# Lemok00/IDEAS

Measured on AMD Instinct MI355X. Metric: train images/sec at 256x256 (G+D+Ex step), higher is better.
Workload: dtype f32; 1 GPU; IDEAS N=1 sigma=1 256x256 batch=32/GPU full G+D+Ex iteration (lazy R1 every 16, EMA), full-width nets, HIP kernels (BASELINE.json configs[2]); global_batch=32, parallelism=dp1, r1_steps_in_window=0, ranks=1

## Files before the change

### ideas_amd/csrc/conv_b3_wgrad3.hip

```cpp
#include "b3.hpp"
#include "conv_launch.hpp"

ideas_plan ideas_b3_wgrad3_plan(const ideas_conv_params* p, int, int64_t slots) {
    if (slots <= 0) slots = 512;
    const int64_t tiles = (int64_t)(p->Cout / 64) * (p->Cin / 64), strips = p->OW / 16, rows_total = (int64_t)p->B * p->OH;
    const int64_t spl = std::min(splitk_target(slots, tiles * strips, rows_total, 128), std::max<int64_t>(rows_total / 16, 1));
    const SplitK k = splitk_round(rows_total, spl, 1);
    return {{k.splits * strips, k.per}, slots};
}

namespace {

typedef short s16x4 __attribute__((ext_vector_type(4)));
typedef short s16x8 __attribute__((ext_vector_type(8)));

template <int S> struct W3 {
    static constexpr int XW = 15 * S + 3;
    static constexpr int NR = 4;
    static constexpr int XROWS = NR * XW;
    static constexpr int GROWS = 2 * 16;
    static constexpr int XPLANE = XROWS * 128, GPLANE = GROWS * 128;
    static constexpr int LDS = 3 * (XPLANE + GPLANE);
    static constexpr int XLOADS = (XW * 16 + 255) / 256;
};


template <int S, bool SCALE, bool REFLECT>
__global__ __launch_bounds__(256, 2) void conv_b3_wgrad3_kernel(float* __restrict__ gw, const float* __restrict__ gy,
                                                                const float* __restrict__ x, const float* __restrict__ in_scale,
                                                                const float* __restrict__ out_scale, ideas_conv_params p,
                                                                int tiles_ci, int tiles, int splits, int strips, int rows_per_split,
                                                                unsigned gy_bytes, unsigned x_bytes) {
    using L = W3<S>;
    constexpr int XW = L::XW, NR = L::NR;
    __shared__ __attribute__((aligned(16))) unsigned char smem[L::LDS];
    unsigned char* const sG = smem;
    unsigned char* const sX = smem + 3 * L::GPLANE;

    const int t = threadIdx.x, lane = t & 63, wave = t >> 6;
    int tile, split;
    splitk_xcd_map(blockIdx.x, tiles, splits, tile, split);
    const int o0 = (tile / tiles_ci) * 64, c0 = (tile % tiles_ci) * 64;
    const int strip = split % strips, range = split / strips;
    const int ox0 = strip * 16;
    const int rows_total = p.B * p.OH;
    const int R0 = range * rows_per_split;
    const int R1 = R0 + rows_per_split < rows_total ? R0 + rows_per_split : rows_total;
    if (R0 >= R1) return;

    const __amdgpu_buffer_rsrc_t rg = __builtin_amdgcn_make_buffer_rsrc((void*)gy, 0, (int)gy_bytes, (int)RSRC_FLAGS);
    const __amdgpu_buffer_rsrc_t rx = __builtin_amdgcn_make_buffer_rsrc((void*)x, 0, (int)x_bytes, (int)RSRC_FLAGS);
    const __amdgpu_buffer_rsrc_t rso = __builtin_amdgcn_make_buffer_rsrc((void*)out_scale, 0, SCALE ? p.B * p.Cout * 4 : 0, (int)RSRC_FLAGS);
    const __amdgpu_buffer_rsrc_t rsi = __builtin_amdgcn_make_buffer_rsrc((void*)in_scale, 0, SCALE ? p.B * p.Cin * 4 : 0, (int)RSRC_FLAGS);

    const int quad = t & 15, px = t >> 4;
    const unsigned g_cb = (unsigned)(o0 + quad * 4) * 4u, x_cb = (unsigned)(c0 + quad * 4) * 4u;
    auto xrow_of = [](int j) { return S == 1 ? j : (j & 1) * 17 + (j >> 1); };
    int x_lrow[L::XLOADS];
    bool x_on[L::XLOADS];
#pragma unroll
    for (int k = 0; k < L::XLOADS; ++k) {
        const int j = px + 16 * k;
        x_on[k] = j < XW;
        x_lrow[k] = xrow_of(j < XW ? j : 0);
    }

    struct Task { int b, wy, oy; bool mma, live; };
    int tk_b, tk_oa, tk_ob, tk_wy, tk_g;
    bool tk_done = false;
    {
        tk_g = R0;
        tk_b = R0 / p.OH;
        tk_oa = R0 - tk_b * p.OH;
        const int left = R1 - R0;
        tk_ob = tk_oa + left < p.OH ? tk_oa + left : p.OH;
        tk_wy = tk_oa * S;
    }
    auto next_task = [&]() -> Task {
        Task k;
        k.live = !tk_done;
        k.b = tk_b;
        k.wy = tk_wy;
        const int rel = tk_wy - tk_oa * S;
        k.mma = k.live && rel >= 2 && ((rel - 2) % S == 0);
        k.oy = tk_oa + (rel - 2) / S;
        if (!tk_done) {
            ++tk_wy;
            if (tk_wy > (tk_ob - 1) * S + 2) {
                tk_g += tk_ob - tk_oa;
                if (tk_g >= R1) tk_done = true;
                else {
                    ++tk_b;
                    tk_oa = 0;
                    tk_ob = R1 - tk_g < p.OH ? R1 - tk_g : p.OH;
                    tk_wy = 0;
                }
            }
        }
        return k;
    };

    struct Stage { float4 g, xv[L::XLOADS], sg, sx; };
    auto gload = [&](Stage& st, const Task& k) {
        int iy = k.wy + p.offy;
        bool yok = k.live;
        if (REFLECT) iy = reflect_coord(iy, p.IH);
        else yok = yok && (unsigned)iy < (unsigned)p.IH;
        const unsigned rowb = (unsigned)((k.b * p.IH + iy) * p.IW) * (unsigned)p.Cin * 4u + x_cb;
#pragma unroll
        for (int q = 0; q < L::XLOADS; ++q) {
            int ix = ox0 * S + p.offx + px + 16 * q;
            bool ok = yok && x_on[q];
            if (REFLECT) ix = reflect_coord(ix, p.IW);
            else ok = ok && (unsigned)ix < (unsigned)p.IW;
            st.xv[q] = buffer_load4(rx, ok ? rowb + (unsigned)ix * (unsigned)p.Cin * 4u : 0xffffffffu, 0);
        }
        const unsigned goff = (unsigned)(((k.b * p.OH + k.oy) * p.OW + ox0 + px) * p.Cout) * 4u + g_cb;
        st.g = buffer_load4(rg, k.mma ? goff : 0xffffffffu, 0);
        if (SCALE) {
            st.sg = buffer_load4(rso, (unsigned)(k.b * p.Cout) * 4u + g_cb, 0);
            st.sx = buffer_load4(rsi, (unsigned)(k.b * p.Cin) * 4u + x_cb, 0);
        }
    };
    auto put = [&](unsigned char* plane0, int plane_bytes, int row, float4 v, float4 sc) {
        if (SCALE) v = b3_scale4(v, sc);
        const Split4 s = split4(v);
        unsigned char* a = plane0 + chunk_off(row, quad >> 1) + (quad & 1) * 8;
#pragma unroll
        for (int pl = 0; pl < 3; ++pl) *reinterpret_cast<uint2*>(a + pl * plane_bytes) = s.p[pl];
    };
    auto lstore = [&](const Stage& st, int n) {
        const int slot = n % NR;
#pragma unroll
        for (int q = 0; q < L::XLOADS; ++q)
            if (x_on[q]) put(sX, L::XPLANE, slot * XW + x_lrow[q], st.xv[q], st.sx);
        put(sG, L::GPLANE, (n & 1) * 16 + px, st.g, st.sg);
    };

    const int wo = wave >> 1, wc = wave & 1;
    const int li = lane & 31, lh = lane >> 5;
    const int g_q = lane & 15, g_row = g_q >> 2, g_piece = g_q & 3, g_cblk = (lane >> 4) & 1;
    auto lane_base = [&](unsigned region, int b, int cb) {
        const int r = b + 8 * lh + g_row;
        return region + (unsigned)(r * 128 + (((cb * 2 + (g_piece >> 1)) ^ ((((b + g_row) >> 1) & 1) << 2)) << 4) + (g_piece & 1) * 8);
    };
    const unsigned ldsG = (unsigned)(uintptr_t)(__attribute__((address_space(3))) unsigned char*)sG;
    const unsigned ldsX = (unsigned)(uintptr_t)(__attribute__((address_space(3))) unsigned char*)sX;
    unsigned baseG[4], baseX[4];
#pragma unroll
    for (int b = 0; b < 4; ++b) { baseG[b] = lane_base(ldsG, b, wo * 2 + g_cblk); baseX[b] = lane_base(ldsX, b, wc * 2 + g_cblk); }
    auto tr_ld = [&](unsigned addr) -> s16x4 {
        return __builtin_amdgcn_ds_read_tr16_b64_v4i16((__attribute__((address_space(3))) s16x4*)(uintptr_t)addr);
    };
    auto frag = [&](const unsigned (&base)[4], int plane_off, int r0) -> bf16x8 {
        const unsigned a0 = base[r0 & 3] + (unsigned)(plane_off + (r0 & ~3) * 128);
        const s16x4 a = tr_ld(a0);
        const s16x4 b = tr_ld(a0 + 512u);
        const s16x8 v = {a[0], a[1], a[2], a[3], b[0], b[1], b[2], b[3]};
        return __builtin_bit_cast(bf16x8, v);
    };

    f32x16 acc[9];
#pragma unroll
    for (int a = 0; a < 9; ++a)
#pragma unroll
        for (int r = 0; r < 16; ++r) acc[a][r] = 0.f;

    auto compute = [&](auto ph_) {
        constexpr int PH = decltype(ph_)::value;
        bf16x8 fa[3];
#pragma unroll
        for (int pl = 0; pl < 3; ++pl) fa[pl] = frag(baseG, pl * L::GPLANE, (PH & 1) * 16);
        auto loadB = [&](int tap, bf16x8 (&fb)[3]) {
            const int ty = tap / 3, tx = tap - 3 * ty;
            const int r0 = ((PH + 2 + ty) % NR) * XW + (S == 1 ? tx : (tx & 1) * 17 + (tx >> 1));
#pragma unroll
            for (int pl = 0; pl < 3; ++pl) fb[pl] = frag(baseX, pl * L::XPLANE, r0);
        };
        bf16x8 fb[5][2][3];
        loadB(0, fb[0][0]);
        loadB(1, fb[0][1]);
#pragma unroll
        for (int pr = 0; pr < 5; ++pr) {
            if (pr < 4) {
                loadB(2 * pr + 2, fb[pr + 1][0]);
                if (2 * pr + 3 < 9) loadB(2 * pr + 3, fb[pr + 1][1]);
            }
            __builtin_amdgcn_sched_barrier(0);
#pragma unroll
            for (int q = 0; q < 6; ++q) {
                acc[2 * pr] = __builtin_amdgcn_mfma_f32_32x32x16_bf16(fa[PA[q]], fb[pr][0][PB[q]], acc[2 * pr], 0, 0, 0);
                if (2 * pr + 1 < 9)
                    acc[2 * pr + 1] = __builtin_amdgcn_mfma_f32_32x32x16_bf16(fa[PA[q]], fb[pr][1][PB[q]], acc[2 * pr + 1], 0, 0, 0);
            }
            __builtin_amdgcn_sched_barrier(0);
        }
    };

    Stage st0, st1;
    Task k0 = next_task();
    gload(st0, k0);
    Task k1 = next_task();
    gload(st1, k1);
    lstore(st0, 0);
    __syncthreads();
    bool mma0 = k0.mma, mma1 = k1.mma, live0 = k0.live, live1 = k1.live;
    static_assert(NR == 4, "the step loop is unrolled over the ring positions");
    auto step = [&](auto ph_, Stage& ld, const Stage& stg) {
        constexpr int PH = decltype(ph_)::value;
        const Task k2 = next_task();
        gload(ld, k2);
        if (live1) lstore(stg, PH + 1);
        if (mma0) compute(ph_);
        __syncthreads();
        mma0 = mma1; live0 = live1; mma1 = k2.mma; live1 = k2.live;
    };
    while (live0) {
        step(std::integral_constant<int, 0>{}, st0, st1);
        if (!live0) break;
        step(std::integral_constant<int, 1>{}, st1, st0);
        if (!live0) break;
        step(std::integral_constant<int, 2>{}, st0, st1);
        if (!live0) break;
        step(std::integral_constant<int, 3>{}, st1, st0);
    }

    const int ci = c0 + wc * 32 + li;
#pragma unroll
    for (int tap = 0; tap < 9; ++tap)
#pragma unroll
        for (int r = 0; r < 16; ++r) {
            const int o = o0 + wo * 32 + (r & 3) + 8 * (r >> 2) + 4 * lh;
            atomicAdd(&gw[((int64_t)o * 9 + tap) * p.Cin + ci], acc[tap][r] * p.gain);
        }
}



template <int S>
int launch_wgrad3(float* gw, const void* gy, const void* x, const float* in_scale, const float* out_scale, const ideas_conv_params* p,
                  hipStream_t stream) {
    const int tiles_ci = p->Cin / 64, tiles = (p->Cout / 64) * tiles_ci;
    const int strips = p->OW / 16;
    const SplitK k = ideas_b3_wgrad3_plan(p, 0, 0).k;
    if (!ideas_grid_fits(tiles * k.splits)) return IDEAS_E_SHAPE;
    with_flags(in_scale && out_scale, p->reflect, [&](auto sc, auto rf) {
        hipLaunchKernelGGL((conv_b3_wgrad3_kernel<S, decltype(sc)::value, decltype(rf)::value>), dim3(splitk_grid(tiles, k.splits)),
                           dim3(256), 0, stream, gw, (const float*)gy, (const float*)x, in_scale, out_scale, *p, tiles_ci, tiles,
                           (int)k.splits, strips, (int)k.per, ideas_gy_bytes(p, 4), ideas_x_bytes(p, 4));
    });
    return ideas_launch_status();
}

}

bool ideas_b3_wgrad3_enabled() { return !ideas_env_off("IDEAS_B3_WGRAD3"); }

extern "C" int ideas_b3_wgrad3_supported(const ideas_conv_params* p) {
    if (!p) return 0;
    if (p->TY != 3 || p->TX != 3 || p->dy != 1 || p->dx != 1 || p->sy != p->sx || (p->sy != 1 && p->sy != 2)) return 0;
    if (p->osy != 1 || p->osx != 1 || p->ooy != 0 || p->oox != 0 || p->YH != p->OH || p->YW != p->OW) return 0;
    if (p->OW % 16 || p->Cin % 64 || p->Cout % 64) return 0;
    if (p->sy == 2 && ideas_env_off("IDEAS_B3_WGRAD3_S2")) return 0;
    if (p->reflect && (p->IH < 2 || p->IW < 2)) return 0;
    if (p->offx > 0 || p->offx < -2 || p->offy > 0 || p->offy < -2) return 0;
    return (int64_t)p->B * p->IH * p->IW * p->Cin * 4 < 0xffffffffLL && (int64_t)p->B * p->YH * p->YW * p->Cout * 4 < 0xffffffffLL &&
           (int64_t)p->B * p->OH < 0x7fffffffLL;
}

int ideas_b3_wgrad3(float* gw, const void* gy, const void* x, const float* in_scale, const float* out_scale, const ideas_conv_params* p,
                    hipStream_t stream) {
    if (p->sy == 1) return launch_wgrad3<1>(gw, gy, x, in_scale, out_scale, p, stream);
    return launch_wgrad3<2>(gw, gy, x, in_scale, out_scale, p, stream);
}
```

Before: 85.74 images/sec.

## Extend 3x3 weight-grad MFMA kernel to narrow widths and 32-channel inputs

Adds new tilings to the 3x3 weight-gradient kernel. Small spatial widths (8 or 4 pixels) pack several images into one 16-pixel strip. Layers with Cin=32 use a pair of 16-pixel strips so the 64-wide tile stays full. Before this, these shapes fell back to a generic weight-grad path. The change adds several template instantiations and layout complexity, and the narrow-width case with scaling still routes to the old kernel.

```diff
diff --git a/ideas_amd/csrc/conv_b3_wgrad3.hip b/ideas_amd/csrc/conv_b3_wgrad3.hip
--- a/ideas_amd/csrc/conv_b3_wgrad3.hip
+++ b/ideas_amd/csrc/conv_b3_wgrad3.hip
@@ -1,9 +1,18 @@
 #include "b3.hpp"
 #include "conv_launch.hpp"
 
+enum { W3_WIDE = 16, W3_PAIR = 32, W3_SEG8 = 8, W3_SEG4 = 4 };
+static int w3_form(const ideas_conv_params* p) {
+    if (p->Cin == 32) return W3_PAIR;
+    return p->OW == 8 ? W3_SEG8 : p->OW == 4 ? W3_SEG4 : W3_WIDE;
+}
+
 ideas_plan ideas_b3_wgrad3_plan(const ideas_conv_params* p, int, int64_t slots) {
     if (slots <= 0) slots = 512;
-    const int64_t tiles = (int64_t)(p->Cout / 64) * (p->Cin / 64), strips = p->OW / 16, rows_total = (int64_t)p->B * p->OH;
+    const int form = w3_form(p);
+    const int64_t tiles = (int64_t)(p->Cout / 64) * (form == W3_PAIR ? 1 : p->Cin / 64);
+    const int64_t strips = form == W3_PAIR ? std::max(p->OW / 32, 1) : form == W3_WIDE ? p->OW / 16 : 1;
+    const int64_t rows_total = (form == W3_SEG8 || form == W3_SEG4 ? (int64_t)p->B / (16 / form) : (int64_t)p->B) * p->OH;
     const int64_t spl = std::min(splitk_target(slots, tiles * strips, rows_total, 128), std::max<int64_t>(rows_total / 16, 1));
     const SplitK k = splitk_round(rows_total, spl, 1);
     return {{k.splits * strips, k.per}, slots};
@@ -14,25 +23,37 @@
 typedef short s16x4 __attribute__((ext_vector_type(4)));
 typedef short s16x8 __attribute__((ext_vector_type(8)));
 
-template <int S> struct W3 {
-    static constexpr int XW = 15 * S + 3;
+template <int S, int SEG = 16, bool PAIR = false> struct W3 {
+    static constexpr int NIMG = 16 / SEG;
+    static constexpr int SW = (SEG - 1) * S + 3;
+    static constexpr int EVEN = SEG + 1;
+    static constexpr int PITCH = (SEG == 4 && S == 1) ? 8 : SW;
+    static constexpr bool BASE2 = SEG == 4 && PITCH % 4 != 0;
+    static constexpr int XW = NIMG * PITCH;
+    static constexpr int XSTAGED = NIMG * SW;
     static constexpr int NR = 4;
     static constexpr int XROWS = NR * XW;
-    static constexpr int GROWS = 2 * 16;
+    static constexpr int GPIX = PAIR ? 32 : 16;
+    static constexpr int GROWS = 2 * GPIX;
     static constexpr int XPLANE = XROWS * 128, GPLANE = GROWS * 128;
     static constexpr int LDS = 3 * (XPLANE + GPLANE);
-    static constexpr int XLOADS = (XW * 16 + 255) / 256;
+    static constexpr int XLOADS = (XSTAGED * 16 + 255) / 256;
+    static_assert(LDS <= 80 * 1024, "two blocks per CU");
 };
 
 
-template <int S, bool SCALE, bool REFLECT>
+template <int S, bool SCALE, bool REFLECT, int SEG = 16, bool PAIR = false>
 __global__ __launch_bounds__(256, 2) void conv_b3_wgrad3_kernel(float* __restrict__ gw, const float* __restrict__ gy,
                                                                 const float* __restrict__ x, const float* __restrict__ in_scale,
                                                                 const float* __restrict__ out_scale, ideas_conv_params p,
                                                                 int tiles_ci, int tiles, int splits, int strips, int rows_per_split,
                                                                 unsigned gy_bytes, unsigned x_bytes) {
-    using L = W3<S>;
+    using L = W3<S, SEG, PAIR>;
     constexpr int XW = L::XW, NR = L::NR;
+    constexpr bool WIDE = SEG == 16 && !PAIR;
+    static_assert(SEG == 16 || SEG == 8 || SEG == 4, "a strip is 16 pixels");
+    static_assert(!PAIR || (SEG == 16 && S == 1), "strip pairs: stride 1");
+    static_assert(SEG == 16 || !SCALE, "image groups: unscaled");
     __shared__ __attribute__((aligned(16))) unsigned char smem[L::LDS];
     unsigned char* const sG = smem;
     unsigned char* const sX = smem + 3 * L::GPLANE;
@@ -42,8 +63,8 @@
     splitk_xcd_map(blockIdx.x, tiles, splits, tile, split);
     const int o0 = (tile / tiles_ci) * 64, c0 = (tile % tiles_ci) * 64;
     const int strip = split % strips, range = split / strips;
-    const int ox0 = strip * 16;
-    const int rows_total = p.B * p.OH;
+    const int ox0 = strip * (PAIR ? 32 : 16);
+    const int rows_total = (SEG < 16 ? p.B / L::NIMG : p.B) * p.OH;
     const int R0 = range * rows_per_split;
     const int R1 = R0 + rows_per_split < rows_total ? R0 + rows_per_split : rows_total;
     if (R0 >= R1) return;
@@ -54,15 +75,34 @@
     const __amdgpu_buffer_rsrc_t rsi = __builtin_amdgcn_make_buffer_rsrc((void*)in_scale, 0, SCALE ? p.B * p.Cin * 4 : 0, (int)RSRC_FLAGS);
 
     const int quad = t & 15, px = t >> 4;
-    const unsigned g_cb = (unsigned)(o0 + quad * 4) * 4u, x_cb = (unsigned)(c0 + quad * 4) * 4u;
-    auto xrow_of = [](int j) { return S == 1 ? j : (j & 1) * 17 + (j >> 1); };
+    const unsigned g_cb = (unsigned)(o0 + quad * 4) * 4u, x_cb = (unsigned)(c0 + (PAIR ? quad & 7 : quad) * 4) * 4u;
+    auto xrow_of = [](int j) { return S == 1 ? j : (j & 1) * L::EVEN + (j >> 1); };
     int x_lrow[L::XLOADS];
     bool x_on[L::XLOADS];
-#pragma unroll
-    for (int k = 0; k < L::XLOADS; ++k) {
-        const int j = px + 16 * k;
-        x_on[k] = j < XW;
-        x_lrow[k] = xrow_of(j < XW ? j : 0);
+    bool x_ok[L::XLOADS];
+    unsigned x_voff[L::XLOADS], g_voff = 0;
+    if constexpr (WIDE) {
+#pragma unroll
+        for (int k = 0; k < L::XLOADS; ++k) {
+            const int j = px + 16 * k;
+            x_on[k] = j < XW;
+            x_lrow[k] = xrow_of(j < XW ? j : 0);
+        }
+    } else {
+#pragma unroll
+        for (int k = 0; k < L::XLOADS; ++k) {
+            const int j = px + 16 * k;
+            x_on[k] = j < L::XSTAGED;
+            const int jj = x_on[k] ? j : 0, img = jj / L::SW, col = jj - img * L::SW;
+            x_lrow[k] = img * L::PITCH + xrow_of(col);
+            int ix = (PAIR ? ox0 + 16 * (quad >> 3) : 0) + p.offx + col;
+            x_ok[k] = x_on[k];
+            if (REFLECT) ix = reflect_coord(ix, p.IW);
+            else x_ok[k] = x_ok[k] && (unsigned)ix < (unsigned)p.IW;
+            x_voff[k] = (unsigned)(img * p.IH * p.IW + ix) * (unsigned)p.Cin * 4u + x_cb;
+        }
+        const int g_pix = PAIR ? ox0 + px : (px / SEG) * p.OH * p.OW + px % SEG;
+        g_voff = (unsigned)(g_pix * p.Cout) * 4u + g_cb;
     }
 
     struct Task { int b, wy, oy; bool mma, live; };
@@ -100,23 +140,33 @@
         return k;
     };
 
-    struct Stage { float4 g, xv[L::XLOADS], sg, sx; };
+    struct Stage { float4 g[PAIR ? 2 : 1], xv[L::XLOADS], sg, sx; };
     auto gload = [&](Stage& st, const Task& k) {
         int iy = k.wy + p.offy;
         bool yok = k.live;
         if (REFLECT) iy = reflect_coord(iy, p.IH);
         else yok = yok && (unsigned)iy < (unsigned)p.IH;
-        const unsigned rowb = (unsigned)((k.b * p.IH + iy) * p.IW) * (unsigned)p.Cin * 4u + x_cb;
-#pragma unroll
-        for (int q = 0; q < L::XLOADS; ++q) {
-            int ix = ox0 * S + p.offx + px + 16 * q;
-            bool ok = yok && x_on[q];
-            if (REFLECT) ix = reflect_coord(ix, p.IW);
-            else ok = ok && (unsigned)ix < (unsigned)p.IW;
-            st.xv[q] = buffer_load4(rx, ok ? rowb + (unsigned)ix * (unsigned)p.Cin * 4u : 0xffffffffu, 0);
-        }
-        const unsigned goff = (unsigned)(((k.b * p.OH + k.oy) * p.OW + ox0 + px) * p.Cout) * 4u + g_cb;
-        st.g = buffer_load4(rg, k.mma ? goff : 0xffffffffu, 0);
+        if constexpr (WIDE) {
+            const unsigned rowb = (unsigned)((k.b * p.IH + iy) * p.IW) * (unsigned)p.Cin * 4u + x_cb;
+#pragma unroll
+            for (int q = 0; q < L::XLOADS; ++q) {
+                int ix = ox0 * S + p.offx + px + 16 * q;
+                bool ok = yok && x_on[q];
+                if (REFLECT) ix = reflect_coord(ix, p.IW);
+                else ok = ok && (unsigned)ix < (unsigned)p.IW;
+                st.xv[q] = buffer_load4(rx, ok ? rowb + (unsigned)ix * (unsigned)p.Cin * 4u : 0xffffffffu, 0);
+            }
+            const unsigned goff = (unsigned)(((k.b * p.OH + k.oy) * p.OW + ox0 + px) * p.Cout) * 4u + g_cb;
+            st.g[0] = buffer_load4(rg, k.mma ? goff : 0xffffffffu, 0);
+        } else {
+            const int b0 = SEG < 16 ? k.b * L::NIMG : k.b;
+            const unsigned rowb = (unsigned)((b0 * p.IH + iy) * p.IW) * (unsigned)p.Cin * 4u;
+#pragma unroll
+            for (int q = 0; q < L::XLOADS; ++q) st.xv[q] = buffer_load4(rx, yok && x_ok[q] ? rowb + x_voff[q] : 0xffffffffu, 0);
+            const unsigned goff = (unsigned)(((b0 * p.OH + k.oy) * p.OW) * p.Cout) * 4u + g_voff;
+            st.g[0] = buffer_load4(rg, k.mma ? goff : 0xffffffffu, 0);
+            if constexpr (PAIR) st.g[1] = buffer_load4(rg, k.mma ? goff + (unsigned)(16 * p.Cout) * 4u : 0xffffffffu, 0);
+        }
         if (SCALE) {
             st.sg = buffer_load4(rso, (unsigned)(k.b * p.Cout) * 4u + g_cb, 0);
             st.sx = buffer_load4(rsi, (unsigned)(k.b * p.Cin) * 4u + x_cb, 0);
@@ -134,7 +184,8 @@
 #pragma unroll
         for (int q = 0; q < L::XLOADS; ++q)
             if (x_on[q]) put(sX, L::XPLANE, slot * XW + x_lrow[q], st.xv[q], st.sx);
-        put(sG, L::GPLANE, (n & 1) * 16 + px, st.g, st.sg);
+        put(sG, L::GPLANE, (n & 1) * L::GPIX + px, st.g[0], st.sg);
+        if constexpr (PAIR) put(sG, L::GPLANE, (n & 1) * L::GPIX + 16 + px, st.g[1], st.sg);
     };
 
     const int wo = wave >> 1, wc = wave & 1;
@@ -146,9 +197,24 @@
     };
     const unsigned ldsG = (unsigned)(uintptr_t)(__attribute__((address_space(3))) unsigned char*)sG;
     const unsigned ldsX = (unsigned)(uintptr_t)(__attribute__((address_space(3))) unsigned char*)sX;
-    unsigned baseG[4], baseX[4];
-#pragma unroll
-    for (int b = 0; b < 4; ++b) { baseG[b] = lane_base(ldsG, b, wo * 2 + g_cblk); baseX[b] = lane_base(ldsX, b, wc * 2 + g_cblk); }
+    auto lane_base_seg = [&](unsigned region, int b, int cb, int off) {
+        const int r = b + off + g_row;
+        return region + (unsigned)(r * 128 + (((cb * 2 + (g_piece >> 1)) ^ (((r >> 1) & 1) << 2)) << 4) + (g_piece & 1) * 8);
+    };
+    constexpr int LH_ROWS = SEG == 16 ? 8 : SEG == 8 ? L::PITCH : 2 * L::PITCH;
+    constexpr int BLK2_ROWS = SEG == 4 ? L::PITCH : 4;
+    unsigned baseG[4], baseX[4], baseX2[4];
+#pragma unroll
+    for (int b = 0; b < 4; ++b) {
+        if constexpr (WIDE) {
+            baseG[b] = lane_base(ldsG, b, wo * 2 + g_cblk);
+            baseX[b] = lane_base(ldsX, b, wc * 2 + g_cblk);
+        } else {
+            baseG[b] = lane_base(ldsG + (PAIR ? wc * 16 * 128 : 0), b, wo * 2 + g_cblk);
+            baseX[b] = lane_base_seg(ldsX, b, wc * 2 + g_cblk, LH_ROWS * lh);
+            if constexpr (L::BASE2) baseX2[b] = lane_base_seg(ldsX, b, wc * 2 + g_cblk, LH_ROWS * lh + BLK2_ROWS);
+        }
+    }
     auto tr_ld = [&](unsigned addr) -> s16x4 {
         return __builtin_amdgcn_ds_read_tr16_b64_v4i16((__attribute__((address_space(3))) s16x4*)(uintptr_t)addr);
     };
@@ -159,6 +225,13 @@
         const s16x8 v = {a[0], a[1], a[2], a[3], b[0], b[1], b[2], b[3]};
         return __builtin_bit_cast(bf16x8, v);
     };
+    auto frag_seg = [&](int plane_off, int r0) -> bf16x8 {
+        const unsigned imm = (unsigned)(plane_off + (r0 & ~3) * 128);
+        const s16x4 a = tr_ld(baseX[r0 & 3] + imm);
+        const s16x4 b = tr_ld(L::BASE2 ? baseX2[r0 & 3] + imm : baseX[r0 & 3] + imm + (unsigned)(BLK2_ROWS * 128));
+        const s16x8 v = {a[0], a[1], a[2], a[3], b[0], b[1], b[2], b[3]};
+        return __builtin_bit_cast(bf16x8, v);
+    };
 
     f32x16 acc[9];
 #pragma unroll
@@ -170,12 +243,15 @@
         constexpr int PH = decltype(ph_)::value;
         bf16x8 fa[3];
 #pragma unroll
-        for (int pl = 0; pl < 3; ++pl) fa[pl] = frag(baseG, pl * L::GPLANE, (PH & 1) * 16);
+        for (int pl = 0; pl < 3; ++pl) fa[pl] = frag(baseG, pl * L::GPLANE, (PH & 1) * L::GPIX);
         auto loadB = [&](int tap, bf16x8 (&fb)[3]) {
             const int ty = tap / 3, tx = tap - 3 * ty;
-            const int r0 = ((PH + 2 + ty) % NR) * XW + (S == 1 ? tx : (tx & 1) * 17 + (tx >> 1));
-#pragma unroll
-            for (int pl = 0; pl < 3; ++pl) fb[pl] = frag(baseX, pl * L::XPLANE, r0);
+            const int r0 = ((PH + 2 + ty) % NR) * XW + (S == 1 ? tx : (tx & 1) * L::EVEN + (tx >> 1));
+#pragma unroll
+            for (int pl = 0; pl < 3; ++pl) {
+                if constexpr (SEG == 16) fb[pl] = frag(baseX, pl * L::XPLANE, r0);
+                else fb[pl] = frag_seg(pl * L::XPLANE, r0);
+            }
         };
         bf16x8 fb[5][2][3];
         loadB(0, fb[0][0]);
@@ -225,7 +301,7 @@
         step(std::integral_constant<int, 3>{}, st1, st0);
     }
 
-    const int ci = c0 + wc * 32 + li;
+    const int ci = c0 + (PAIR ? 0 : wc * 32) + li;
 #pragma unroll
     for (int tap = 0; tap < 9; ++tap)
 #pragma unroll
@@ -237,17 +313,18 @@
 
 
 
-template <int S>
+template <int S, int SEG = 16, bool PAIR = false>
 int launch_wgrad3(float* gw, const void* gy, const void* x, const float* in_scale, const float* out_scale, const ideas_conv_params* p,
                   hipStream_t stream) {
-    const int tiles_ci = p->Cin / 64, tiles = (p->Cout / 64) * tiles_ci;
-    const int strips = p->OW / 16;
+    const int tiles_ci = PAIR ? 1 : p->Cin / 64, tiles = (p->Cout / 64) * tiles_ci;
+    const int strips = PAIR ? p->OW / 32 : SEG < 16 ? 1 : p->OW / 16;
     const SplitK k = ideas_b3_wgrad3_plan(p, 0, 0).k;
     if (!ideas_grid_fits(tiles * k.splits)) return IDEAS_E_SHAPE;
     with_flags(in_scale && out_scale, p->reflect, [&](auto sc, auto rf) {
-        hipLaunchKernelGGL((conv_b3_wgrad3_kernel<S, decltype(sc)::value, decltype(rf)::value>), dim3(splitk_grid(tiles, k.splits)),
-                           dim3(256), 0, stream, gw, (const float*)gy, (const float*)x, in_scale, out_scale, *p, tiles_ci, tiles,
-                           (int)k.splits, strips, (int)k.per, ideas_gy_bytes(p, 4), ideas_x_bytes(p, 4));
+        if constexpr (SEG == 16 || !decltype(sc)::value)
+            hipLaunchKernelGGL((conv_b3_wgrad3_kernel<S, decltype(sc)::value, decltype(rf)::value, SEG, PAIR>),
+                               dim3(splitk_grid(tiles, k.splits)), dim3(256), 0, stream, gw, (const float*)gy, (const float*)x, in_scale,
+                               out_scale, *p, tiles_ci, tiles, (int)k.splits, strips, (int)k.per, ideas_gy_bytes(p, 4), ideas_x_bytes(p, 4));
     });
     return ideas_launch_status();
 }
@@ -260,7 +337,15 @@
     if (!p) return 0;
     if (p->TY != 3 || p->TX != 3 || p->dy != 1 || p->dx != 1 || p->sy != p->sx || (p->sy != 1 && p->sy != 2)) return 0;
     if (p->osy != 1 || p->osx != 1 || p->ooy != 0 || p->oox != 0 || p->YH != p->OH || p->YW != p->OW) return 0;
-    if (p->OW % 16 || p->Cin % 64 || p->Cout % 64) return 0;
+    const int form = w3_form(p);
+    if (form == W3_WIDE) {
+        if (p->OW % 16 || p->Cin % 64 || p->Cout % 64) return 0;
+    } else {
+        if (ideas_env_off("IDEAS_B3_WGRAD3_NARROW") || p->Cout % 64) return 0;
+        if (form == W3_PAIR) {
+            if (p->OW % 32 || p->sy != 1) return 0;
+        } else if (p->Cin % 64 || p->B % (16 / form) || p->OH < 16 / form) return 0;
+    }
     if (p->sy == 2 && ideas_env_off("IDEAS_B3_WGRAD3_S2")) return 0;
     if (p->reflect && (p->IH < 2 || p->IW < 2)) return 0;
     if (p->offx > 0 || p->offx < -2 || p->offy > 0 || p->offy < -2) return 0;
@@ -270,6 +355,16 @@
 
 int ideas_b3_wgrad3(float* gw, const void* gy, const void* x, const float* in_scale, const float* out_scale, const ideas_conv_params* p,
                     hipStream_t stream) {
+    const int form = w3_form(p);
+    if (form == W3_PAIR) return launch_wgrad3<1, 16, true>(gw, gy, x, in_scale, out_scale, p, stream);
+    if (form != W3_WIDE) {
+        if (in_scale && out_scale) return ideas_b3_wgrad(gw, gy, x, in_scale, out_scale, p, stream);
+        if (form == W3_SEG8)
+            return p->sy == 1 ? launch_wgrad3<1, 8>(gw, gy, x, in_scale, out_scale, p, stream)
+                              : launch_wgrad3<2, 8>(gw, gy, x, in_scale, out_scale, p, stream);
+        return p->sy == 1 ? launch_wgrad3<1, 4>(gw, gy, x, in_scale, out_scale, p, stream)
+                          : launch_wgrad3<2, 4>(gw, gy, x, in_scale, out_scale, p, stream);
+    }
     if (p->sy == 1) return launch_wgrad3<1>(gw, gy, x, in_scale, out_scale, p, stream);
     return launch_wgrad3<2>(gw, gy, x, in_scale, out_scale, p, stream);
 }
```

New measurement: 86.39 images/sec (median of 6 runs). No clear change (+0.8%).
